# lavajuno/afskmodem

Measured on AMD Instinct MI355X. Metric: Msamples/s demodulated (batched 48 kHz streams) + decoded-byte match rate vs CPU ref, higher is better.
Workload: dtype int16

## Files before the change

### afskmodem_amd/csrc/afsk_live_stream.hip

```cpp

namespace afsk {

struct StreamDemod {
    int32_t phase;
    int32_t ci;
    int32_t k;
    int32_t first;
    int32_t nbits;
    int32_t corrected;
    uint32_t bits;
    int32_t spare;
};
static_assert(sizeof(StreamDemod) == 32, "StreamDemod layout");

constexpr int kStreamWin = 2 * kListenBlock;
constexpr int kStreamWinLds = 2 * kStreamWin + 128;

struct LiveStreamLayout {
    int64_t n = 0, slots = 0, max_payload = 0;
    int64_t o_carry = 0, o_demod = 0, o_bf = 0, o_win = 0, o_pay = 0, bytes = 0;
};

inline int live_stream_layout(int32_t n_channels, int32_t max_payload_len, int32_t max_chunk_len, LiveStreamLayout& L,
                              bool per_channel = false) {
    if (n_channels < 1) return fail(AFSK_E_INVALID_ARG, "n_channels must be at least 1");
    if (max_payload_len < 0 || max_payload_len > 65536)
        return fail(AFSK_E_INVALID_ARG, "max_payload_len must lie in 0 ... 65536");
    if (max_chunk_len < 1 || max_chunk_len > kMaxStreamLen)
        return fail(AFSK_E_INVALID_ARG, "max_chunk_len must lie in 1 ... AFSK_MAX_STREAM_LEN");
    const int64_t k_blocks = ((int64_t)kListenBlock - 1 + max_chunk_len) / kListenBlock;
    L.n = n_channels;
    L.slots = 1 + k_blocks / 3;
    L.max_payload = max_payload_len;
    if (L.n * L.slots > 0x7fffffffll)
        return fail(AFSK_E_INVALID_ARG, "n_channels * slots exceeds the demodulator's int32 stream count");
    L.o_carry = align256(32 * L.n);
    L.o_demod = L.o_carry + align256(2 * kListenBlock * L.n);
    L.o_bf = L.o_demod + align256(32 * L.n);
    L.o_win = L.o_bf + align256((per_channel ? 12 : 4) * L.n);
    L.o_pay = L.o_win + align256(2 * kStreamWin * L.n);
    L.bytes = L.o_pay + align256(L.max_payload * L.n) + 256;
    return AFSK_OK;
}

struct LiveStreamArgs {
    LiveArgs g;
    StreamDemod* dm;
    const int32_t* bit_frames;
    int16_t* win;
    uint8_t* pay;
    int32_t max_payload;
    uint8_t* out_bytes;
    int32_t out_stride;
    int32_t* out_nbytes;
    int32_t* out_nbits;
    int32_t* out_clock_idx;
    int32_t* out_term_frame;
    int32_t* out_status;
    int32_t* out_corrected;
};

__device__ __forceinline__ void stream_symbols(const int16_t* win, int lane, int bf, int lsh, int32_t s0, int n,
                                               uint32_t amp_thr, uint64_t& dec, uint64_t& loud) {
    const int lps = 1 << lsh;
    const int g = lane >> lsh, sub = lane & (lps - 1);
    const bool valid = g < n;
    const int32_t base = s0 + (valid ? g : 0) * bf;
    const int q = bf >> 2;
    int32_t sm = 0, ss = 0;
    uint32_t amp = 0;
    int qi = 0, nb = q;
    for (int j = sub; j < bf; j += lps) {
        if (j >= nb) { qi++; nb += q; }
        const int32_t x = win[(base + j) & (kStreamWin - 1)];
        const int32_t h = x > 512 ? 0 : (x < -512 ? 65535 : 32767);
        sm += (qi & 1) ? -h : h;
        ss += (qi & 2) ? -h : h;
        amp += (uint32_t)(x < 0 ? -x : x);
    }
    for (int m = lps >> 1; m > 0; m >>= 1) {
        sm += __shfl_xor(sm, m);
        ss += __shfl_xor(ss, m);
        amp += (uint32_t)__shfl_xor((int)amp, m);
    }
    const uint32_t full = 65535u * (uint32_t)q;
    const uint32_t md = (2u * full + (uint32_t)sm) / (uint32_t)bf, sd = (2u * full + (uint32_t)ss) / (uint32_t)bf;
    int r = (md < sd ? 1 : 0) | (amp >= amp_thr ? 2 : 0);
    if (lsh > 0) r = __shfl(r, (lane < n ? lane : 0) << lsh);
    dec = __ballot(lane < n && (r & 1));
    loud = __ballot(lane < n && (r & 2));
}

struct LiveStreamSink {
    const LiveStreamArgs& A;
    int16_t* lwin;
    StreamDemod ds;
    int bf, lsh;
    uint32_t amp_thr;
    int16_t* gwin;
    uint8_t* pay;

    __device__ __forceinline__ void init(const LiveArgs&, int c, int32_t amp_end) {
        ds = A.dm[c];
        bf = A.bit_frames[c];
        int l = 0;
        while ((2 << l) * 32 <= bf) l++;
        lsh = l;
        amp_thr = split_amp_thr(amp_end, bf);
        gwin = A.win + (int64_t)c * kStreamWin;
        pay = A.pay + (int64_t)c * A.max_payload;
    }
    __device__ __forceinline__ void copy_tail(bool out, int64_t from, int64_t to, int lane) {
        for (int64_t p = from + lane; p < to; p += 64) {
            const int i = (int)(p & (kStreamWin - 1));
            if (out) gwin[i] = lwin[i];
            else lwin[i] = gwin[i];
        }
    }
    __device__ __forceinline__ bool live_demod(const LiveChan& st) const {
        return st.mode == 2 && ds.phase < 3 && st.rec_len <= kMaxStreamLen;
    }
    __device__ __forceinline__ int64_t tail_from(const LiveChan& st) const {
        return ds.phase == 0 ? 0 : (int64_t)ds.ci + (int64_t)ds.k * bf;
    }
    __device__ __forceinline__ void begin(const LiveArgs&, int lane, const LiveChan& st) {
        if (live_demod(st)) copy_tail(false, tail_from(st), st.rec_len, lane);
        wave_lds_sync();
    }
    __device__ __forceinline__ bool overflowed(const LiveArgs&, const LiveChan& st) const {
        return st.rec_len > kMaxStreamLen;
    }
    __device__ __forceinline__ void slot(const LiveArgs&, int64_t, int, const LiveChan&, bool) const {}
    __device__ __forceinline__ void report(const LiveArgs&, int64_t i, const LiveChan& st, bool ovf, int32_t, int lane) {
        int32_t status, nbits = 0, ci = -1, term = -1, corrected = 0;
        if (ovf) status = AFSK_ST_BAD_LENGTH;
        else if (ds.phase == 0) status = AFSK_ST_TOO_SHORT;
        else {
            ci = ds.ci;
            if (ds.phase == 1) term = ds.ci + ds.k * bf;
            else {
                term = ds.ci + ds.first * bf;
                nbits = ds.nbits;
                corrected = ds.corrected;
            }
            status = nbits == 0 ? AFSK_ST_NO_DATA : AFSK_ST_OK;
        }
        const int32_t nbytes = (nbits / 7) >> 1;
        if (lane == 0) {
            A.out_nbytes[i] = nbytes;
            A.out_nbits[i] = nbits;
            A.out_clock_idx[i] = ci;
            A.out_term_frame[i] = term;
            A.out_status[i] = status;
            if (A.out_corrected) A.out_corrected[i] = corrected;
        }
        int32_t nb = nbytes < A.max_payload ? nbytes : A.max_payload;
        nb = nb < A.out_stride ? nb : A.out_stride;
        if (nb > 0) {
            __builtin_amdgcn_fence(__ATOMIC_SEQ_CST, "workgroup");
            uint8_t* row = A.out_bytes + i * A.out_stride;
            for (int b = lane; b < nb; b += 64) row[b] = pay[b];
        }
    }
    __device__ __forceinline__ void start(const LiveChan&) { ds = StreamDemod{}; }

    __device__ __forceinline__ void step(uint32_t d, uint32_t l, int m, int32_t k0, int lane) {
        int s = 0;
        if (ds.phase == 1) {
            const uint64_t ext = ((uint64_t)d << 3) | (ds.bits & 7u);
            const uint64_t hit = ext & ~(ext >> 1) & ~(ext >> 2) & ~(ext >> 3) & ((1ull << m) - 1ull);
            if (!hit) {
                ds.bits = (uint32_t)(ext >> m) & 7u;
                return;
            }
            const int t = __builtin_ctzll(hit);
            ds.first = k0 + t + 1;
            ds.phase = 2;
            ds.bits = 0;
            s = t + 1;
        }
        const int r = m - s;
        if (r <= 0) return;
        const uint32_t mask = r >= 32 ? ~0u : ((1u << r) - 1u);
        const uint32_t quiet = ~(l >> s) & mask;
        int take = r;
        if (quiet) {
            take = __builtin_ctz(quiet);
            ds.phase = 3;
        }
        if (take == 0) return;
        const uint32_t tmask = take >= 32 ? ~0u : ((1u << take) - 1u);
        int have = ds.nbits % 7;
        int32_t cw_index = ds.nbits / 7;
        uint64_t acc = (uint64_t)(ds.bits & 0x7Fu) | ((uint64_t)((d >> s) & tmask) << have);
        uint32_t hi = (ds.bits >> 8) & 0xFu;
        ds.nbits += take;
        have += take;
        while (have >= 7) {
            const uint32_t cw = (uint32_t)acc & 0x7Fu;
            acc >>= 7;
            have -= 7;
            ds.corrected += hamming_syndrome(cw) != 0u;
            const uint32_t nib = hamming_nibble(cw);
            if (cw_index & 1) {
                const int32_t b = cw_index >> 1;
                if (b < A.max_payload && lane == 0) pay[b] = (uint8_t)((hi << 4) | nib);
            } else {
                hi = nib;
            }
            cw_index++;
        }
        ds.bits = ((uint32_t)acc & 0x7Fu) | (hi << 8);
    }

    __device__ __forceinline__ void record(const LiveArgs&, const LiveChan& st, const vec16 (&cur)[4], int lane) {
        if (!live_demod(st) || st.rec_len + kListenBlock > kMaxStreamLen) return;
        const int32_t jb = (int32_t)(st.rec_len >> 11);
        uint8_t* half = reinterpret_cast<uint8_t*>(lwin) + (jb & 1) * (2 * kListenBlock);
        wave_lds_sync();
#pragma unroll
        for (int j = 0; j < 4; j++) *reinterpret_cast<vec16*>(half + 1024 * j + 16 * lane) = cur[j];
        wave_lds_sync();
        if (jb == 0) return;
        if (ds.phase == 0) {
            FastRing fr;
            fr.ring = reinterpret_cast<uint8_t*>(lwin);
            fr.lane = lane;
            fr.next = 8;
            fr.warm_ops = 0;
            int ci;
            if (bf == 40) {
                if (clock_index_is_zero<40, 8>(fr)) ci = 0;
                else ci = recover_clock_index_lanes<40, false, 8>(fr);
            } else {
                ci = recover_clock_index_rt(fr, bf);
            }
            ds.ci = ci;
            ds.k = 0;
            ds.phase = 1;
            ds.bits = 0;
            wave_lds_sync();
        }
        const int32_t len = (int32_t)st.rec_len + kListenBlock;
        const int32_t k_end = (len - ds.ci - 1) / bf;
        const int spp = 64 >> lsh;
        while (ds.k < k_end && ds.phase < 3) {
            const int n = k_end - ds.k < spp ? k_end - ds.k : spp;
            uint64_t dec, loud;
            stream_symbols(lwin, lane, bf, lsh, ds.ci + ds.k * bf, n, amp_thr, dec, loud);
            for (int h = 0; h < n && ds.phase < 3; h += 32) {
                const int m = n - h < 32 ? n - h : 32;
                step((uint32_t)(dec >> h), (uint32_t)(loud >> h), m, ds.k + h, lane);
            }
            ds.k += n;
        }
    }
    __device__ __forceinline__ int32_t head(const LiveChan&) const { return 0; }
    __device__ __forceinline__ void finish(const LiveArgs&, int c, const LiveChan& st, int lane) {
        wave_lds_sync();
        if (live_demod(st)) copy_tail(true, tail_from(st), st.rec_len, lane);
        if (lane == 0) A.dm[c] = ds;
    }
    __device__ __forceinline__ void clear(const LiveArgs&, int64_t slot0, int i) const {
        const int64_t s = slot0 + i;
        A.out_nbytes[s] = 0;
        A.out_nbits[s] = 0;
        A.out_clock_idx[s] = -1;
        A.out_term_frame[s] = -1;
        A.out_status[s] = AFSK_ST_TOO_SHORT;
        if (A.out_corrected) A.out_corrected[s] = 0;
    }
};

__global__ __launch_bounds__(256) void live_stream_kernel(LiveStreamArgs a) {
    __shared__ __attribute__((aligned(16))) uint8_t lds[4 * kStreamWinLds];
    LiveStreamSink sk{a, reinterpret_cast<int16_t*>(lds + (threadIdx.x >> 6) * kStreamWinLds)};
    live_gate_walk(a.g, sk);
}

__global__ __launch_bounds__(256) void live_stream_thr_kernel(LiveStreamArgs a, const int32_t* thr_start,
                                                              const int32_t* thr_end) {
    __shared__ __attribute__((aligned(16))) uint8_t lds[4 * kStreamWinLds];
    LiveStreamSink sk{a, reinterpret_cast<int16_t*>(lds + (threadIdx.x >> 6) * kStreamWinLds)};
    live_gate_walk<true>(a.g, sk, thr_start, thr_end);
}

__global__ __launch_bounds__(256) void live_stream_reset_kernel(LiveChan* chan, StreamDemod* dm, const uint8_t* mask,
                                                                int32_t n) {
    const int c = blockIdx.x * 256 + threadIdx.x;
    if (c < n && (!mask || mask[c])) {
        chan[c] = LiveChan{};
        dm[c] = StreamDemod{};
    }
}

}

namespace afsk {

int live_stream_push(afsk_live* live, const int16_t* chunk, int64_t chunk_row_stride, int32_t chunk_len, int32_t flush,
                     int32_t* out_n_closed, int64_t* out_burst_start, int32_t* out_burst_len, int32_t* out_flags,
                     const DemodOutputs& o, hipStream_t stream) {
    LiveStreamLayout L;
    if (int rc = live_stream_layout((int32_t)live->L.n, live->max_payload_len, live->max_chunk_len, L, live->per_channel))
        return rc;
    uint8_t* d = live->state.ptr();
    LiveStreamArgs a{};
    a.g.chan = reinterpret_cast<LiveChan*>(d);
    a.g.carry = reinterpret_cast<int16_t*>(d + L.o_carry);
    a.g.chunk = chunk_len > 0 ? chunk : a.g.carry;
    a.g.chunk_stride = chunk_len > 0 ? chunk_row_stride : 0;
    a.g.chunk_len = chunk_len;
    a.g.flush = flush != 0;
    a.g.n = (int32_t)L.n;
    a.g.slots = (int32_t)L.slots;
    a.g.amp_start = live->amp_start;
    a.g.amp_end = live->amp_end;
    a.g.out_n_closed = out_n_closed;
    a.g.out_burst_start = out_burst_start;
    a.g.out_burst_len = out_burst_len;
    a.g.out_flags = out_flags;
    a.dm = reinterpret_cast<StreamDemod*>(d + L.o_demod);
    a.bit_frames = reinterpret_cast<const int32_t*>(d + L.o_bf);
    a.win = reinterpret_cast<int16_t*>(d + L.o_win);
    a.pay = d + L.o_pay;
    a.max_payload = (int32_t)L.max_payload;
    a.out_bytes = o.bytes;
    a.out_stride = o.stride;
    a.out_nbytes = o.nbytes;
    a.out_nbits = o.nbits;
    a.out_clock_idx = o.clock_idx;
    a.out_term_frame = o.term_frame;
    a.out_status = o.status;
    a.out_corrected = o.corrected;
    if (live->per_channel)
        hipLaunchKernelGGL(live_stream_thr_kernel, dim3((uint32_t)((L.n + 3) / 4)), dim3(256), 0, stream, a,
                           live->thr_start(), live->thr_end());
    else
        hipLaunchKernelGGL(live_stream_kernel, dim3((uint32_t)((L.n + 3) / 4)), dim3(256), 0, stream, a);
    hipError_t e = hipGetLastError();
    return e == hipSuccess ? AFSK_OK
                           : hip_fail(e, live->per_channel ? "launch live_stream_thr_kernel" : "launch live_stream_kernel");
}

int live_stream_reset(afsk_live* live, const uint8_t* d_mask_or_null, hipStream_t stream) {
    LiveStreamLayout L;
    if (int rc = live_stream_layout((int32_t)live->L.n, live->max_payload_len, live->max_chunk_len, L, live->per_channel))
        return rc;
    uint8_t* d = live->state.ptr();
    hipLaunchKernelGGL(live_stream_reset_kernel, dim3((uint32_t)((L.n + 255) / 256)), dim3(256), 0, stream,
                       reinterpret_cast<LiveChan*>(d), reinterpret_cast<StreamDemod*>(d + L.o_demod), d_mask_or_null,
                       (int32_t)L.n);
    hipError_t e = hipGetLastError();
    return e == hipSuccess ? AFSK_OK : hip_fail(e, "launch live_stream_reset_kernel");
}

int live_stream_state(const LiveSpec& sp, afsk_live& lv) {
    LiveStreamLayout L;
    if (int rc = live_stream_layout(sp.n_channels, sp.max_payload_len, sp.max_chunk_len, L, sp.per_channel)) return rc;
    lv.L.n = L.n;
    lv.L.slots = L.slots;
    lv.bit_frames = 0;
    lv.max_payload_len = sp.max_payload_len;
    std::vector<int32_t> up(sp.bit_frames, sp.bit_frames + L.n);
    if (sp.per_channel) {
        lv.o_thr = L.o_bf + 4 * L.n;
        up.insert(up.end(), sp.amp_start, sp.amp_start + L.n);
        up.insert(up.end(), sp.amp_end, sp.amp_end + L.n);
    }
    return lv.state.create(sp.entry, L.bytes, L.o_bf, up.data(), L.o_bf, 4 * (int64_t)up.size());
}

}

extern "C" {

int afsk_live_stream_layout(int32_t n_channels, int32_t max_payload_len, int32_t max_chunk_len, int32_t* out_slots,
                            int64_t* out_state_bytes) {
    afsk::LiveStreamLayout L;
    if (int rc = afsk::live_stream_layout(n_channels, max_payload_len, max_chunk_len, L)) return rc;
    if (out_slots) *out_slots = (int32_t)L.slots;
    if (out_state_bytes) *out_state_bytes = L.bytes;
    return AFSK_OK;
}

int afsk_live_create_stream(int32_t n_channels, const int32_t* bit_frames_host, int32_t amp_start_threshold,
                            int32_t amp_end_threshold, int32_t max_payload_len, int32_t max_chunk_len, afsk_live** out) {
    bool same;
    if (int rc = live_check_rates(n_channels, bit_frames_host, out, same)) return rc;
    return live_create({"afsk_live_create_stream", n_channels, bit_frames_host, true, &amp_start_threshold,
                        &amp_end_threshold, false, true, 0, max_payload_len, max_chunk_len}, out);
}

int afsk_live_create_stream_thresholds(int32_t n_channels, const int32_t* bit_frames_host, const int32_t* amp_start_host,
                                       const int32_t* amp_end_host, int32_t max_payload_len, int32_t max_chunk_len,
                                       afsk_live** out) {
    bool same;
    if (int rc = live_check_rates(n_channels, bit_frames_host, out, same)) return rc;
    if (!amp_start_host || !amp_end_host) return afsk::fail(AFSK_E_INVALID_ARG, "null pointer argument");
    const bool per_channel = !all_equal(amp_start_host, n_channels) || !all_equal(amp_end_host, n_channels);
    return live_create({"afsk_live_create_stream_thresholds", n_channels, bit_frames_host, true, amp_start_host,
                        amp_end_host, per_channel, true, 0, max_payload_len, max_chunk_len}, out);
}

}
```

Baseline: 3.786 million.

## Vectorize stream symbol demod with SAD ops, mirrored LDS window, new clock recovery

Replaces the per-sample scalar symbol integrator with a bf=40 specialization that loads the window as 128-bit words and uses SAD/alignbyte packed-16 arithmetic, plus a generic packed-pair path for other frame sizes. Adds a 128-byte mirror past the LDS ring so vector loads need no wraparound masking. Replaces the FastRing clock recovery with a DPP-scan based sliding correlation, and forces demod state to be wave-uniform via readfirstlane. The goal is to cut per-sample VALU and LDS work and scalarize control flow, at the cost of more code, more registers and the risk of bit-exactness mismatches.

```diff
diff --git a/afskmodem_amd/csrc/afsk_live_stream.hip b/afskmodem_amd/csrc/afsk_live_stream.hip
--- a/afskmodem_amd/csrc/afsk_live_stream.hip
+++ b/afskmodem_amd/csrc/afsk_live_stream.hip
@@ -60,24 +60,79 @@
     int32_t* out_corrected;
 };
 
-__device__ __forceinline__ void stream_symbols(const int16_t* win, int lane, int bf, int lsh, int32_t s0, int n,
-                                               uint32_t amp_thr, uint64_t& dec, uint64_t& loud) {
+__device__ __forceinline__ int32_t uni(int32_t v) { return __builtin_amdgcn_readfirstlane(v); }
+__device__ __forceinline__ int64_t uni64(int64_t v) {
+    return (int64_t)(((uint64_t)(uint32_t)uni((int32_t)((uint64_t)v >> 32)) << 32) | (uint32_t)uni((int32_t)v));
+}
+
+constexpr int kStreamMirror = 128;
+
+template <int A, bool ODD>
+__device__ __forceinline__ void stream_symbols_40(const uint8_t* win, int lane, int32_t s0, int n, uint32_t amp_thr,
+                                                  uint64_t& dec, uint64_t& loud) {
+    constexpr int BF = 40, Q = BF / 4;
+    constexpr uint32_t FULL = 65535u;
+    const uint8_t* src = win + ((2 * (s0 + BF * lane)) & (2 * kStreamWin - 16));
+    constexpr int NW = A + 20 + (ODD ? 1 : 0);
+    uint32_t W[24];
+#pragma unroll
+    for (int i = 0; i < 6; i++) {
+        if (4 * i < NW) {
+            const u32x4 t = *reinterpret_cast<const u32x4*>(src + 16 * i);
+            W[4 * i] = t[0]; W[4 * i + 1] = t[1]; W[4 * i + 2] = t[2]; W[4 * i + 3] = t[3];
+        } else {
+            W[4 * i] = W[4 * i + 1] = W[4 * i + 2] = W[4 * i + 3] = 0;
+        }
+    }
+    uint32_t x[20];
+#pragma unroll
+    for (int d = 0; d < 20; d++) x[d] = ODD ? __builtin_amdgcn_alignbyte(W[A + d + 1], W[A + d], 2) : W[A + d];
+    const uint32_t h0 = hi_sad<0, 5>(x), h1 = hi_sad<5, 10>(x), h2 = hi_sad<10, 15>(x), h3 = hi_sad<15, 20>(x);
+    const uint32_t mark = 2u * FULL * Q + h0 + h2 - h1 - h3;
+    const uint32_t space = 2u * FULL * Q + h0 + h1 - h2 - h3;
+    const uint32_t md = mark / (uint32_t)BF, sd = space / (uint32_t)BF;
+    dec = __ballot(lane < n && md < sd);
+    loud = __ballot(lane < n && loud_enough(quiet_sum<0, 20>(x), (uint32_t)BF, amp_thr));
+}
+
+__device__ __forceinline__ void stream_symbols_40(const uint8_t* win, int lane, int32_t s0, int n, uint32_t amp_thr,
+                                                  uint64_t& dec, uint64_t& loud) {
+    switch ((2 * s0) & 15) {
+        case 0: stream_symbols_40<0, false>(win, lane, s0, n, amp_thr, dec, loud); break;
+        case 2: stream_symbols_40<0, true>(win, lane, s0, n, amp_thr, dec, loud); break;
+        case 4: stream_symbols_40<1, false>(win, lane, s0, n, amp_thr, dec, loud); break;
+        case 6: stream_symbols_40<1, true>(win, lane, s0, n, amp_thr, dec, loud); break;
+        case 8: stream_symbols_40<2, false>(win, lane, s0, n, amp_thr, dec, loud); break;
+        case 10: stream_symbols_40<2, true>(win, lane, s0, n, amp_thr, dec, loud); break;
+        case 12: stream_symbols_40<3, false>(win, lane, s0, n, amp_thr, dec, loud); break;
+        default: stream_symbols_40<3, true>(win, lane, s0, n, amp_thr, dec, loud); break;
+    }
+}
+
+__device__ __forceinline__ void stream_symbols_rt(const uint8_t* win, int lane, int bf, int lsh, int32_t s0, int n,
+                                                  uint32_t amp_thr, uint64_t& dec, uint64_t& loud) {
     const int lps = 1 << lsh;
     const int g = lane >> lsh, sub = lane & (lps - 1);
     const bool valid = g < n;
     const int32_t base = s0 + (valid ? g : 0) * bf;
-    const int q = bf >> 2;
-    int32_t sm = 0, ss = 0;
-    uint32_t amp = 0;
-    int qi = 0, nb = q;
-    for (int j = sub; j < bf; j += lps) {
-        if (j >= nb) { qi++; nb += q; }
-        const int32_t x = win[(base + j) & (kStreamWin - 1)];
-        const int32_t h = x > 512 ? 0 : (x < -512 ? 65535 : 32767);
-        sm += (qi & 1) ? -h : h;
-        ss += (qi & 2) ? -h : h;
-        amp += (uint32_t)(x < 0 ? -x : x);
-    }
+    const uint32_t* w32 = reinterpret_cast<const uint32_t*>(win);
+    const uint32_t sh = (s0 & 1) ? 16u : 0u;
+    const int w0 = base >> 1;
+    const int q = bf >> 2, D = bf >> 1;
+    uint32_t T = 0, P = 0, S = 0, amp = 0;
+    for (int d = sub; d < D; d += lps) {
+        const int i = (w0 + d) & (kStreamWin / 2 - 1);
+        const uint32_t x = __builtin_amdgcn_alignbit(w32[i + 1], w32[i], sh);
+        const uint32_t lim = limit_pair_biased(x);
+        const bool second = d >= q;
+        const int e2 = 2 * (second ? d - q : d);
+        const uint32_t odd_mask = (e2 < q ? 0x0000FFFFu : 0u) | (e2 + 1 < q ? 0xFFFF0000u : 0u);
+        T = __builtin_amdgcn_sad_u16(lim, 0xFFFFFFFFu, T);
+        P = __builtin_amdgcn_sad_u16(lim | odd_mask, 0xFFFFFFFFu, P);
+        S = __builtin_amdgcn_sad_u16(second ? lim : 0xFFFFFFFFu, 0xFFFFFFFFu, S);
+        amp = __builtin_amdgcn_sad_u16(x ^ kBias, kBias, amp);
+    }
+    int32_t sm = (int32_t)(T - 2u * P), ss = (int32_t)(T - 2u * S);
     for (int m = lps >> 1; m > 0; m >>= 1) {
         sm += __shfl_xor(sm, m);
         ss += __shfl_xor(ss, m);
@@ -89,6 +144,74 @@
     if (lsh > 0) r = __shfl(r, (lane < n ? lane : 0) << lsh);
     dec = __ballot(lane < n && (r & 1));
     loud = __ballot(lane < n && (r & 2));
+}
+
+__device__ __forceinline__ int stream_clock_index(const uint8_t* win, int lane, int bf) {
+    constexpr int GC = 8, STEP = 64 * GC;
+    const int N = 2 * bf, q = bf >> 2, h = bf >> 1, NOFF = kSync - N;
+    uint32_t base;
+    {
+        const float rcp_q = 1.0f / (float)q;
+        int32_t a = 0;
+        for (int m = lane; m < bf; m += 64) {
+            const uint32_t w = *reinterpret_cast<const uint32_t*>(win + 4 * m);
+            uint32_t cf = 0;
+#pragma unroll
+            for (int half = 0; half < 2; half++) {
+                const int j = 2 * m + half;
+                const bool hi = j < bf ? ((div_exact((uint32_t)j, (uint32_t)q, rcp_q) & 1u) == 0) : ((j - bf) < h);
+                cf |= (hi ? 0xFFFFu : 0x0001u) << (16 * half);
+            }
+            a = dot2_i16(w, cf, a);
+        }
+        base = 65535u * (uint32_t)bf + (uint32_t)__builtin_amdgcn_readlane(wave_incl_scan_dpp(a), 63);
+    }
+    const int steps = (NOFF + STEP - 1) / STEP;
+    const int lag[7] = {0, q, 2 * q, 3 * q, bf, bf + h, N};
+    constexpr int coef[7] = {1, -2, 2, -2, 2, -2, 1};
+    const float rcp_n = 1.0f / (float)N;
+    uint32_t lane_bound = 0xFFFFFFFFu, lane_key = 0xFFFFFFFFu;
+    for (int t = 0; t < steps; t++) {
+        const int f = STEP * t + GC * lane;
+        const int fa = f < NOFF ? f : NOFF - 2;
+        const uint8_t* src = win + 2 * fa;
+        uint32_t R[7][GC / 2];
+#pragma unroll
+        for (int e = 0; e < 7; e++) {
+            const uint8_t* p = src + 2 * (lag[e] & ~1);
+            const uint32_t sh = (lag[e] & 1) ? 2u : 0u;
+            uint32_t W[GC / 2 + 1];
+#pragma unroll
+            for (int j = 0; j <= GC / 2; j++) W[j] = *reinterpret_cast<const uint32_t*>(p + 4 * j);
+#pragma unroll
+            for (int j = 0; j < GC / 2; j++) R[e][j] = __builtin_amdgcn_alignbyte(W[j + 1], W[j], sh);
+        }
+        int32_t run[GC];
+        int32_t acc = 0;
+#pragma unroll
+        for (int k = 0; k < GC; k++) {
+#pragma unroll
+            for (int e = 0; e < 7; e++) {
+                const uint32_t c = (uint32_t)(uint16_t)(int16_t)coef[e];
+                acc = dot2_i16(R[e][k >> 1], (k & 1) ? (c << 16) : c, acc);
+            }
+            run[k] = acc;
+        }
+        const int32_t incl = wave_incl_scan_dpp(acc);
+        const uint32_t first = base + (uint32_t)(incl - acc);
+        base += (uint32_t)__builtin_amdgcn_readlane(incl, 63);
+#pragma unroll
+        for (int k = 0; k < GC; k++) {
+            const uint32_t tot = k == 0 ? first : first + (uint32_t)run[k - 1];
+            const int i = f + k;
+            if (i < NOFF && tot < lane_bound) {
+                const uint32_t mean = div_exact(tot, (uint32_t)N, rcp_n);
+                lane_bound = mean * (uint32_t)N;
+                lane_key = (mean << 12) | (uint32_t)i;
+            }
+        }
+    }
+    return (int)(wave_min_u32(lane_key) & 4095u);
 }
 
 struct LiveStreamSink {
@@ -101,20 +224,34 @@
     uint8_t* pay;
 
     __device__ __forceinline__ void init(const LiveArgs&, int c, int32_t amp_end) {
-        ds = A.dm[c];
-        bf = A.bit_frames[c];
+        const int cu = uni(c);
+        const StreamDemod d = A.dm[cu];
+        ds.phase = uni(d.phase);
+        ds.ci = uni(d.ci);
+        ds.k = uni(d.k);
+        ds.first = uni(d.first);
+        ds.nbits = uni(d.nbits);
+        ds.corrected = uni(d.corrected);
+        ds.bits = (uint32_t)uni((int32_t)d.bits);
+        ds.spare = 0;
+        bf = uni(A.bit_frames[cu]);
         int l = 0;
         while ((2 << l) * 32 <= bf) l++;
         lsh = l;
         amp_thr = split_amp_thr(amp_end, bf);
-        gwin = A.win + (int64_t)c * kStreamWin;
-        pay = A.pay + (int64_t)c * A.max_payload;
+        gwin = A.win + (int64_t)cu * kStreamWin;
+        pay = A.pay + (int64_t)cu * A.max_payload;
     }
     __device__ __forceinline__ void copy_tail(bool out, int64_t from, int64_t to, int lane) {
         for (int64_t p = from + lane; p < to; p += 64) {
             const int i = (int)(p & (kStreamWin - 1));
-            if (out) gwin[i] = lwin[i];
-            else lwin[i] = gwin[i];
+            if (out) {
+                gwin[i] = lwin[i];
+            } else {
+                const int16_t v = gwin[i];
+                lwin[i] = v;
+                if (i < kStreamMirror / 2) lwin[kStreamWin + i] = v;
+            }
         }
     }
     __device__ __forceinline__ bool live_demod(const LiveChan& st) const {
@@ -215,39 +352,43 @@
 
     __device__ __forceinline__ void record(const LiveArgs&, const LiveChan& st, const vec16 (&cur)[4], int lane) {
         if (!live_demod(st) || st.rec_len + kListenBlock > kMaxStreamLen) return;
-        const int32_t jb = (int32_t)(st.rec_len >> 11);
-        uint8_t* half = reinterpret_cast<uint8_t*>(lwin) + (jb & 1) * (2 * kListenBlock);
+        const int32_t rec_len = uni((int32_t)st.rec_len);
+        const int32_t jb = rec_len >> 11;
+        uint8_t* w8 = reinterpret_cast<uint8_t*>(lwin);
+        uint8_t* half = w8 + (jb & 1) * (2 * kListenBlock);
         wave_lds_sync();
 #pragma unroll
         for (int j = 0; j < 4; j++) *reinterpret_cast<vec16*>(half + 1024 * j + 16 * lane) = cur[j];
+        if (!(jb & 1) && lane < kStreamMirror / 16)
+            *reinterpret_cast<vec16*>(w8 + 2 * kStreamWin + 16 * lane) = cur[0];
         wave_lds_sync();
         if (jb == 0) return;
         if (ds.phase == 0) {
-            FastRing fr;
-            fr.ring = reinterpret_cast<uint8_t*>(lwin);
-            fr.lane = lane;
-            fr.next = 8;
-            fr.warm_ops = 0;
-            int ci;
+            int ci = 0;
+            bool zero = false;
             if (bf == 40) {
-                if (clock_index_is_zero<40, 8>(fr)) ci = 0;
-                else ci = recover_clock_index_lanes<40, false, 8>(fr);
-            } else {
-                ci = recover_clock_index_rt(fr, bf);
-            }
-            ds.ci = ci;
+                FastRing fr;
+                fr.ring = w8;
+                fr.lane = lane;
+                fr.next = 8;
+                fr.warm_ops = 0;
+                zero = clock_index_is_zero<40, 8>(fr);
+            }
+            if (!zero) ci = stream_clock_index(w8, lane, bf);
+            ds.ci = uni(ci);
             ds.k = 0;
             ds.phase = 1;
             ds.bits = 0;
             wave_lds_sync();
         }
-        const int32_t len = (int32_t)st.rec_len + kListenBlock;
+        const int32_t len = rec_len + kListenBlock;
         const int32_t k_end = (len - ds.ci - 1) / bf;
         const int spp = 64 >> lsh;
         while (ds.k < k_end && ds.phase < 3) {
             const int n = k_end - ds.k < spp ? k_end - ds.k : spp;
             uint64_t dec, loud;
-            stream_symbols(lwin, lane, bf, lsh, ds.ci + ds.k * bf, n, amp_thr, dec, loud);
+            if (bf == 40) stream_symbols_40(w8, lane, ds.ci + ds.k * 40, n, amp_thr, dec, loud);
+            else stream_symbols_rt(w8, lane, bf, lsh, ds.ci + ds.k * bf, n, amp_thr, dec, loud);
             for (int h = 0; h < n && ds.phase < 3; h += 32) {
                 const int m = n - h < 32 ? n - h : 32;
                 step((uint32_t)(dec >> h), (uint32_t)(loud >> h), m, ds.k + h, lane);
```

Result: no change. 3.786 million, median of 3 (-0.0%).
